# ak110/object_detector

Measured on AMD Instinct MI355X. Metric: images_per_sec, higher is better.
Workload: dtype f16

## Files before the change

object_detector_amd/csrc/conv_8ph_kernel.h:

```cpp
#pragma once
#include "conv_8ph_tile.h"
#include "conv_common.h"

namespace {

constexpr int E_ALO = 0, E_AHI = E_REGION, E_BLO = 2 * E_REGION, E_BHI = 3 * E_REGION;

struct TapWalk {
  int c0, tap, tapoff, dx;
  int sel_tap;
};

constexpr unsigned E_OOB = 0x80000000u;

template <int MT, int NF = 4, bool KEEP = false>
static __device__ __forceinline__ void e8_epilogue_rt(const ConvKP& p, f32x4 (&acc)[MT][NF], int m0w, int n0w, int l15,
                                                          int lq, f16x8 (*keep)[NF / 2] = nullptr, int mrows = MT * 16,
                                                          const float* pre_sc = nullptr, const float* pre_bi = nullptr) {
  unsigned pb[MT], ppix[MT];
#pragma unroll
  for (int i = 0; i < MT; ++i) {
    const int m = m0w + i * 16 + l15;
    pb[i] = (unsigned)m / (unsigned)p.HoWo;
    ppix[i] = (unsigned)m - pb[i] * (unsigned)p.HoWo;
  }
#pragma unroll
  for (int pr = 0; pr < NF / 2; ++pr) {
    const int n = n0w + (2 * pr + (lq & 1)) * 16 + (lq >> 1) * 8;
    const bool nok = n < p.Cout;
    float sc[8], bi[8];
    if (pre_sc) {
#pragma unroll
      for (int e = 0; e < 8; ++e) {
        sc[e] = pre_sc[e];
        bi[e] = pre_bi[e];
      }
    } else {
      const f32x4 s0 = *(const f32x4*)(p.scale + n), s1 = *(const f32x4*)(p.scale + n + 4);
      const f32x4 b0 = *(const f32x4*)(p.bias + n), b1 = *(const f32x4*)(p.bias + n + 4);
#pragma unroll
      for (int e = 0; e < 4; ++e) {
        sc[e] = s0[e];
        sc[4 + e] = s1[e];
        bi[e] = b0[e];
        bi[4 + e] = b1[e];
      }
    }
    f16x8 rv[MT];
#pragma unroll
    for (int i = 0; i < MT; ++i) {
      const int m = m0w + i * 16 + l15;
      f16x8 r = {0, 0, 0, 0, 0, 0, 0, 0};
      if (nok && m < p.M && p.res_mode != OD_RES_NONE) {
        long long roff;
        if (p.res_mode == OD_RES_SAME) {
          roff = (long long)m * p.Cout + n;
        } else {
          const unsigned ho = ppix[i] / (unsigned)p.Wo, wo = ppix[i] - ho * (unsigned)p.Wo;
          roff = ((long long)(pb[i] * (unsigned)(p.Ho >> 1) + (ho >> 1)) * (p.Wo >> 1) + (wo >> 1)) * p.Cout + n;
        }
        r = *(const f16x8*)(p.res + roff);
      }
      rv[i] = r;
    }
#pragma unroll
    for (int i = 0; i < MT; ++i) {
      const int m = m0w + i * 16 + l15;
      const bool ok = nok && m < p.M && i * 16 + l15 < mrows;
      float v[8];
#pragma unroll
      for (int e = 0; e < 4; ++e) {
        float a = acc[i][2 * pr][e], bq = acc[i][2 * pr + 1][e];
        od_permlane16_swap(a, bq);
        v[e] = a;
        v[4 + e] = bq;
      }
#pragma unroll
      for (int e = 0; e < 8; ++e) v[e] = v[e] * sc[e] + bi[e];
      if (p.act == OD_ACT_LEAKY) {
#pragma unroll
        for (int e = 0; e < 8; ++e) v[e] = od_leaky(v[e], p.alpha);
      } else if (p.act == OD_ACT_ELU) {
#pragma unroll
        for (int e = 0; e < 8; ++e) v[e] = v[e] > 0.f ? v[e] : p.alpha * od_expm1_fast(v[e]);
      }
      if (p.res_mode != OD_RES_NONE) {
#pragma unroll
        for (int e = 0; e < 8; ++e) v[e] += (float)rv[i][e];
      }
      if (ok) {
        const long long ooff = (long long)pb[i] * p.obs + (long long)ppix[i] * p.ops + n;
        if (p.out_f32) {
          float* o = (float*)p.out + ooff;
          *(f32x4*)o = f32x4{v[0], v[1], v[2], v[3]};
          *(f32x4*)(o + 4) = f32x4{v[4], v[5], v[6], v[7]};
        } else {
          f16x8 h;
#pragma unroll
          for (int e = 0; e < 8; ++e) h[e] = (f16)v[e];
          *(f16x8*)((f16*)p.out + ooff) = h;
        }
      }
      if (KEEP) {
        f16x8 h;
#pragma unroll
        for (int e = 0; e < 8; ++e) h[e] = (f16)v[e];
        keep[i][pr] = h;
      }
    }
  }
}

template <int EPI, int MT, int NF, bool KEEP>
static __device__ __forceinline__ void e8_epilogue_fixed(const ConvKP& p, f32x4 (&acc)[MT][NF], int m0w, int n0w, int l15, int lq,
                                                         f16x8 (*keep)[NF / 2], int mrows, const float* pre_sc,
                                                         const float* pre_bi) {
  constexpr int ACT = od_epi_act(EPI), RES = od_epi_res(EPI);
  constexpr bool F32 = od_epi_f32(EPI);
  unsigned orow[MT], rrow[RES != OD_RES_NONE ? MT : 1];
#pragma unroll
  for (int i = 0; i < MT; ++i) {
    const unsigned m = (unsigned)min(m0w + i * 16 + l15, p.M - 1);
    const unsigned b = m / (unsigned)p.HoWo, pix = m - b * (unsigned)p.HoWo;
    orow[i] = b * (unsigned)p.obs + pix * (unsigned)p.ops;
    if (RES == OD_RES_SAME) rrow[i] = m * (unsigned)p.Cout;
    if (RES == OD_RES_UP2) {
      const unsigned ho = pix / (unsigned)p.Wo, wo = pix - ho * (unsigned)p.Wo;
      rrow[i] = ((b * (unsigned)(p.Ho >> 1) + (ho >> 1)) * (unsigned)(p.Wo >> 1) + (wo >> 1)) * (unsigned)p.Cout;
    }
  }
#pragma unroll
  for (int pr = 0; pr < NF / 2; ++pr) {
    const int n = n0w + (2 * pr + (lq & 1)) * 16 + (lq >> 1) * 8;
    const bool nok = n < p.Cout;
    float sc[8], bi[8];
    if (pre_sc) {
#pragma unroll
      for (int e = 0; e < 8; ++e) {
        sc[e] = pre_sc[e];
        bi[e] = pre_bi[e];
      }
    } else {
      const f32x4 s0 = *(const f32x4*)(p.scale + n), s1 = *(const f32x4*)(p.scale + n + 4);
      const f32x4 b0 = *(const f32x4*)(p.bias + n), b1 = *(const f32x4*)(p.bias + n + 4);
#pragma unroll
      for (int e = 0; e < 4; ++e) {
        sc[e] = s0[e];
        sc[4 + e] = s1[e];
        bi[e] = b0[e];
        bi[4 + e] = b1[e];
      }
    }
    f16x8 rv[RES != OD_RES_NONE ? MT : 1];
    if (RES != OD_RES_NONE) {
      const unsigned nr = nok ? (unsigned)n : 0u;
#pragma unroll
      for (int i = 0; i < MT; ++i) rv[i] = *(const f16x8*)(p.res + (rrow[i] + nr));
    }
#pragma unroll
    for (int i = 0; i < MT; ++i) {
      f32x4 a = acc[i][2 * pr], bq = acc[i][2 * pr + 1];
      od_permlane16_swap4(a, bq);
      float v[8] = {a[0], a[1], a[2], a[3], bq[0], bq[1], bq[2], bq[3]};
#pragma unroll
      for (int e = 0; e < 8; ++e) v[e] = v[e] * sc[e] + bi[e];
      if (ACT == OD_ACT_LEAKY) {
#pragma unroll
        for (int e = 0; e < 8; ++e) v[e] = od_leaky(v[e], p.alpha);
      } else if (ACT == OD_ACT_ELU) {
#pragma unroll
        for (int e = 0; e < 8; ++e) v[e] = od_elu_select(v[e], p.alpha);
      }
      if (RES != OD_RES_NONE) {
#pragma unroll
        for (int e = 0; e < 8; ++e) v[e] += (float)rv[i][e];
      }
      f16x8 h;
      if (!F32 || KEEP) {
#pragma unroll
        for (int e = 0; e < 8; ++e) h[e] = (f16)v[e];
      }
      if (nok && m0w + i * 16 + l15 < p.M && i * 16 + l15 < mrows) {
        const unsigned ooff = orow[i] + (unsigned)n;
        if (F32) {
          float* o = (float*)p.out + ooff;
          *(f32x4*)o = f32x4{v[0], v[1], v[2], v[3]};
          *(f32x4*)(o + 4) = f32x4{v[4], v[5], v[6], v[7]};
        } else {
          *(f16x8*)((f16*)p.out + ooff) = h;
        }
      }
      if (KEEP) keep[i][pr] = h;
    }
  }
}

template <int MT, int NF = 4, bool KEEP = false, int EPI = OD_EPI_RT>
static __device__ __forceinline__ void e8_epilogue_direct(const ConvKP& p, f32x4 (&acc)[MT][NF], int m0w, int n0w, int l15,
                                                          int lq, f16x8 (*keep)[NF / 2] = nullptr, int mrows = MT * 16,
                                                          const float* pre_sc = nullptr, const float* pre_bi = nullptr) {
  if constexpr (EPI == OD_EPI_RT)
    e8_epilogue_rt<MT, NF, KEEP>(p, acc, m0w, n0w, l15, lq, keep, mrows, pre_sc, pre_bi);
  else
    e8_epilogue_fixed<EPI, MT, NF, KEEP>(p, acc, m0w, n0w, l15, lq, keep, mrows, pre_sc, pre_bi);
}

template <int KS, int MF1, int EPI, int EPI2, bool PW, bool SEG>
__global__ __launch_bounds__(512, 2) void od_conv_8ph(ConvKP p_in) {
  constexpr int MF0 = 4, MT = MF0 + MF1, WROWS = MT * 16, BM = 2 * WROWS;
  extern __shared__ __attribute__((aligned(16))) char smem[];
  const int tid = threadIdx.x;
  const int lane = tid & 63;
  const int wave = __builtin_amdgcn_readfirstlane(tid >> 6);
  const int wr = wave >> 2, wc = wave & 3;
  const int l15 = lane & 15, lq = lane >> 4;

  int logical;
  {
    const int nt = p_in.mtiles * p_in.ntiles;
    const int pid = p_in.splitk > 1 ? (int)blockIdx.x / p_in.splitk : (int)blockIdx.x;
    const int q = nt >> 3, r = nt & 7, xcd = pid & 7, loc = pid >> 3;
    logical = (xcd < r ? xcd * (q + 1) : r * (q + 1) + (xcd - r) * q) + loc;
  }
  int tm = logical / p_in.ntiles;
  const int tn = logical - tm * p_in.ntiles;
  ConvKP p_seg;
  if (SEG) p_seg = p_in;
  if (SEG && p_in.nseg > 1) {
    int sg = 0;
    if (tm >= p_in.seg_tile0[1]) sg = 1;
    if (p_in.nseg > 2 && tm >= p_in.seg_tile0[2]) sg = 2;
    tm -= p_in.seg_tile0[sg];
    p_seg.x = p_in.seg_x[sg];
    p_seg.out = p_in.seg_out[sg];
    p_seg.H = p_seg.Ho = p_in.seg_H[sg];
    p_seg.W = p_seg.Wo = p_in.seg_W[sg];
    p_seg.HoWo = p_seg.H * p_seg.W;
    p_seg.M = p_in.seg_M[sg];
    p_seg.x_bytes = (unsigned)p_seg.M * (unsigned)p_in.Cin * 2u;
    if (p_in.obs == 0) p_seg.obs = (long long)p_seg.HoWo * p_in.Cout;
  }
  const ConvKP& p = SEG ? p_seg : p_in;
  const int m0 = tm * BM, n0 = tn * E_BN;
  const int nk_all = p.Ktot / E_BK;
  const int ks0 = p.splitk > 1 ? ((int)blockIdx.x % p.splitk) * p.steps_per_split : 0;
  const int nk = p.splitk > 1 ? min(p.steps_per_split, nk_all - ks0) : nk_all;
  if (nk <= 0) return;

  const int rr = tid >> 3;
  const int lc = (tid & 7) ^ (rr & 7);
  int a_base[2][2];
  unsigned a_vmask[2][2];
  unsigned a_sel[2][2];
#pragma unroll
  for (int s = 0; s < 2; ++s)
#pragma unroll
    for (int j = 0; j < 2; ++j) {
      const int m = m0 + j * WROWS + s * 64 + rr;
      a_vmask[s][j] = 0u;
      a_base[s][j] = 0;
      if (m < p.M && (s == 0 || rr < MF1 * 16)) {
        const unsigned b = (unsigned)m / (unsigned)p.HoWo;
        const unsigned pix = (unsigned)m - b * (unsigned)p.HoWo;
        const unsigned ho = pix / (unsigned)p.Wo;
        const unsigned wo = pix - ho * (unsigned)p.Wo;
        const int hi0 = (int)ho * p.stride - p.pad, wi0 = (int)wo * p.stride - p.pad;
        a_base[s][j] = ((((int)b * p.H + hi0 + p.pad) * p.W + wi0 + p.pad) * p.Cin + lc * 8) * 2;
#pragma unroll
        for (int t = 0; t < KS * KS; ++t) {
          const int hi = hi0 + t / KS, wi = wi0 + t % KS;
          if ((unsigned)hi < (unsigned)p.H && (unsigned)wi < (unsigned)p.W) a_vmask[s][j] |= 1u << t;
        }
      }
    }
  int w_off[2][2];
#pragma unroll
  for (int s = 0; s < 2; ++s)
#pragma unroll
    for (int j = 0; j < 2; ++j) {
      const int n = n0 + (2 * j + (rr >> 5)) * 64 + s * 32 + (rr & 31);
      w_off[s][j] = (n * p.Kstride + lc * 8 + ks0 * E_BK) * 2;
    }
  const __amdgpu_buffer_rsrc_t rs_x = __builtin_amdgcn_make_buffer_rsrc(
      (void*)(p.x - (long long)p.pad * (p.W + 1) * p.Cin), 0, (int)(p.x_bytes + (unsigned)(p.pad * (p.W + 1) * p.Cin * 2)),
      0x00020000);
  const __amdgpu_buffer_rsrc_t rs_w = __builtin_amdgcn_make_buffer_rsrc((void*)p.w, 0, (int)p.w_bytes, 0x00020000);
  auto blds16 = [&](const __amdgpu_buffer_rsrc_t& rs, unsigned voff, int soff, char* lptr) {
    __builtin_amdgcn_raw_ptr_buffer_load_lds(rs, (__attribute__((address_space(3))) void*)lptr, 16, (int)voff, soff, 0, 0);
  };

  auto walk_init = [&](TapWalk& w, int kt) {
    const int k0 = kt * E_BK;
    if (KS == 3) {
      w.sel_tap = -1;
      w.tap = k0 / p.Cin;
      w.c0 = k0 - w.tap * p.Cin;
      const int dy = w.tap / 3;
      w.dx = w.tap - dy * 3;
      w.tapoff = (dy * p.W + w.dx) * p.Cin;
    } else {
      w.sel_tap = -1;
      w.tap = 0;
      w.c0 = k0;
      w.dx = 0;
      w.tapoff = 0;
    }
  };
  auto walk_next = [&](TapWalk& w) {
    w.c0 += E_BK;
    if (KS == 3 && w.c0 >= p.Cin) {
      w.c0 = 0;
      ++w.tap;
      if (++w.dx == 3) {
        w.dx = 0;
        w.tapoff += (p.W - 2) * p.Cin;
      } else {
        w.tapoff += p.Cin;
      }
    }
  };
  TapWalk walk_lo, walk_hi;
  walk_init(walk_lo, ks0);
  walk_init(walk_hi, ks0);

  char* const piece = smem + wave * 1024;
  auto stage_a = [&](int s, TapWalk& w, int buf) {
    const int koff = w.tapoff + w.c0;
    char* dst = piece + buf * E_BUF + (s ? E_AHI : E_ALO);
    if (w.sel_tap != w.tap) {
      w.sel_tap = w.tap;
#pragma unroll
      for (int j = 0; j < 2; ++j) a_sel[s][j] = ((a_vmask[s][j] >> w.tap) & 1u) ? (unsigned)a_base[s][j] : E_OOB;
    }
#pragma unroll
    for (int j = 0; j < 2; ++j) blds16(rs_x, a_sel[s][j], koff * 2, dst + j * 8192);
    walk_next(w);
  };
  auto stage_b = [&](int s, int t, int buf) {
    char* dst = piece + buf * E_BUF + (s ? E_BHI : E_BLO);
#pragma unroll
    for (int j = 0; j < 2; ++j) blds16(rs_w, (unsigned)w_off[s][j], t * (E_BK * 2), dst + j * 8192);
  };

  const int w2buf = ((nk - 1) & 1) ^ 1;
  const __amdgpu_buffer_rsrc_t rs_w2 =
      __builtin_amdgcn_make_buffer_rsrc((void*)(PW ? p.w2 : p.w), 0, (int)(PW ? p.w2_bytes : p.w_bytes), 0x00020000);
  auto stage_w2 = [&](int ks) {
#pragma unroll
    for (int h = 0; h < 2; ++h)
      blds16(rs_w2, (unsigned)(((h * 64 + rr) * p.K2stride + lc * 8) * 2), ks * (E_BK * 2),
             piece + w2buf * E_BUF + ks * E_REGION + h * 8192);
  };

  f32x4 acc[MT][4];
#pragma unroll
  for (int i = 0; i < MT; ++i)
#pragma unroll
    for (int j = 0; j < 4; ++j) acc[i][j] = f32x4{0.f, 0.f, 0.f, 0.f};

  stage_a(0, walk_lo, 0);
  stage_b(0, 0, 0);
  stage_b(1, 0, 0);
  stage_a(1, walk_hi, 0);
  if (nk > 1) {
    stage_a(0, walk_lo, 1);
    stage_b(0, 1, 1);
    wait_vmcnt<8>();
  } else {
    wait_vmcnt<0>();
  }
  __builtin_amdgcn_s_barrier();

  const int fa = (wr * 64 + l15) * 128 + ((lq ^ (l15 & 7)) * 16);
  const int fb = (wc * 32 + l15) * 128 + ((lq ^ (l15 & 7)) * 16);

  f16x8 xa[MF0][2], wlo[2][2], whi[2][2];
  auto ldf = [&](f16x8& dst, const char* src) { dst = *(const f16x8*)src; };
  auto mma = [&](f32x4& c, const f16x8& a, const f16x8& b) {
    c = __builtin_amdgcn_mfma_f32_16x16x32_f16(a, b, c, 0, 0, 0);
  };

  auto L0 = [&](int t) {
    const char* cur = smem + (t & 1) * E_BUF;
#pragma unroll
    for (int f = 0; f < 2; ++f)
#pragma unroll
      for (int kh = 0; kh < 2; ++kh) ldf(wlo[f][kh], cur + E_BLO + ((fb + f * 2048) ^ (kh * 64)));
#pragma unroll
    for (int f = 0; f < MF0; ++f)
#pragma unroll
      for (int kh = 0; kh < 2; ++kh) ldf(xa[f][kh], cur + E_ALO + ((fa + f * 2048) ^ (kh * 64)));
    if (t + 1 < nk) {
      stage_b(1, t + 1, (t & 1) ^ 1);
      wait_vmcnt<8>();
    } else if (PW) {
      stage_w2(0);
      wait_vmcnt<2>();
    } else {
      wait_vmcnt<0>();
    }
  };
  auto L1 = [&](int t) {
    const char* cur = smem + (t & 1) * E_BUF;
#pragma unroll
    for (int f = 0; f < 2; ++f)
#pragma unroll
      for (int kh = 0; kh < 2; ++kh) ldf(whi[f][kh], cur + E_BHI + ((fb + f * 2048) ^ (kh * 64)));
    if (t + 1 < nk) {
      stage_a(1, walk_hi, (t & 1) ^ 1);
      wait_vmcnt<8>();
    } else if (PW) {
      stage_w2(1);
    } else {
      wait_vmcnt<0>();
    }
  };
  auto L2 = [&](int t) {
    const char* cur = smem + (t & 1) * E_BUF;
#pragma unroll
    for (int f = 0; f < MF1; ++f)
#pragma unroll
      for (int kh = 0; kh < 2; ++kh) ldf(xa[f][kh], cur + E_AHI + ((fa + f * 2048) ^ (kh * 64)));
    if (t + 2 < nk) stage_a(0, walk_lo, t & 1);
    if (PW && t + 1 == nk) stage_w2(2);
  };
  auto L3 = [&](int t) {
    if (t + 2 < nk) {
      stage_b(0, t + 2, t & 1);
      wait_vmcnt<8>();
    } else if (PW && t + 1 == nk) {
      stage_w2(3);
    } else {
      wait_vmcnt<0>();
    }
  };
  auto M = [&](int ph) {
    __builtin_amdgcn_s_setprio(1);
#pragma unroll
    for (int kh = 0; kh < 2; ++kh)
#pragma unroll
      for (int i = 0; i < ((ph < 2) ? MF0 : MF1); ++i)
#pragma unroll
        for (int j = 0; j < 2; ++j) {
          if (ph == 0) mma(acc[i][j], wlo[j][kh], xa[i][kh]);
          if (ph == 1) mma(acc[i][2 + j], whi[j][kh], xa[i][kh]);
          if (ph == 2) mma(acc[MF0 + i][2 + j], whi[j][kh], xa[i][kh]);
          if (ph == 3) mma(acc[MF0 + i][j], wlo[j][kh], xa[i][kh]);
        }
    __builtin_amdgcn_s_setprio(0);
  };

  if (wr == 0) {
    for (int t = 0; t < nk; ++t) {
      L0(t);
      M(0);
      __builtin_amdgcn_s_barrier();
      L1(t);
      M(1);
      __builtin_amdgcn_s_barrier();
      L2(t);
      M(2);
      __builtin_amdgcn_s_barrier();
      L3(t);
      M(3);
      __builtin_amdgcn_s_barrier();
    }
  } else {
    L0(0);
    __builtin_amdgcn_s_barrier();
    for (int t = 0; t < nk; ++t) {
      M(0);
      L1(t);
      __builtin_amdgcn_s_barrier();
      M(1);
      L2(t);
      __builtin_amdgcn_s_barrier();
      M(2);
      L3(t);
      __builtin_amdgcn_s_barrier();
      M(3);
      if (t + 1 < nk) {
        L0(t + 1);
        __builtin_amdgcn_s_barrier();
      }
    }
  }
  __syncthreads();

  if constexpr (PW) {
    const int rg = wave >> 2, cg = wave & 3;
    float sc2[8], bi2[8];
    {
      const int n2 = cg * 32 + (lq & 1) * 16 + (lq >> 1) * 8;
      const f32x4 s0 = *(const f32x4*)(p.scale2 + n2), s1 = *(const f32x4*)(p.scale2 + n2 + 4);
      const f32x4 b0 = *(const f32x4*)(p.bias2 + n2), b1 = *(const f32x4*)(p.bias2 + n2 + 4);
#pragma unroll
      for (int e = 0; e < 4; ++e) {
        sc2[e] = s0[e];
        sc2[4 + e] = s1[e];
        bi2[e] = b0[e];
        bi2[4 + e] = b1[e];
      }
    }
    f16x8 ykeep[MT][2];
    od_mfma_results_ready();
    e8_epilogue_direct<MT, 4, true, EPI>(p, acc, m0 + wr * WROWS, n0 + wc * 64, l15, lq, ykeep);
    ConvKP p2 = p;
    p2.scale = p.scale2;
    p2.bias = p.bias2;
    p2.act = p.act2;
    p2.alpha = p.alpha2;
    p2.res_mode = OD_RES_NONE;
    p2.out = (void*)p.out2;
    p2.out_f32 = 0;
    p2.Cout = p.Cout2;
    p2.obs = (long long)p.HoWo * p.Cout2;
    p2.ops = p.Cout2;
    char* const ybuf = smem + (w2buf ^ 1) * E_BUF;
    const char* const wbuf = smem + w2buf * E_BUF;
    const int fy = (rg * 64 + l15) * 128 + ((lq ^ (l15 & 7)) * 16);
    const int fw = (cg * 32 + l15) * 128 + ((lq ^ (l15 & 7)) * 16);
#pragma unroll
    for (int half = 0; half < 2; ++half) {
      if (wr == half) {
#pragma unroll
        for (int i = 0; i < MT; ++i)
#pragma unroll
          for (int pr = 0; pr < 2; ++pr) {
            const int row = i * 16 + l15;
            const int chunk = (2 * pr + (lq & 1)) * 2 + (lq >> 1);
            *(f16x8*)(ybuf + wc * E_REGION + row * 128 + ((chunk ^ (row & 7)) * 16)) = ykeep[i][pr];
          }
      }
      asm volatile("s_waitcnt lgkmcnt(0)" ::: "memory");
      __builtin_amdgcn_s_barrier();
      f32x4 acc2[4][2];
#pragma unroll
      for (int i = 0; i < 4; ++i)
#pragma unroll
        for (int f = 0; f < 2; ++f) acc2[i][f] = f32x4{0.f, 0.f, 0.f, 0.f};
#pragma unroll
      for (int ks = 0; ks < 4; ++ks)
#pragma unroll
        for (int kh = 0; kh < 2; ++kh) {
          f16x8 wf[2], yf[4];
#pragma unroll
          for (int f = 0; f < 2; ++f) wf[f] = *(const f16x8*)(wbuf + ks * E_REGION + ((fw + f * 2048) ^ (kh * 64)));
#pragma unroll
          for (int i = 0; i < 4; ++i) yf[i] = *(const f16x8*)(ybuf + ks * E_REGION + ((fy + i * 2048) ^ (kh * 64)));
#pragma unroll
          for (int i = 0; i < 4; ++i)
#pragma unroll
            for (int f = 0; f < 2; ++f) acc2[i][f] = __builtin_amdgcn_mfma_f32_16x16x32_f16(wf[f], yf[i], acc2[i][f], 0, 0, 0);
        }
      od_mfma_results_ready();
      e8_epilogue_direct<4, 2, false, EPI2>(p2, acc2, m0 + half * WROWS + rg * 64, cg * 32, l15, lq, nullptr, WROWS - rg * 64, sc2, bi2);
      if (half == 0) {
        asm volatile("s_waitcnt lgkmcnt(0)" ::: "memory");
        __builtin_amdgcn_s_barrier();
      }
    }
  } else if (EPI == OD_EPI_RT && p.splitk > 1) {
    conv_epilogue<E_BN, 2, 4, MT, 4, 512>(p, smem, acc, m0, n0, tid, wr, wc, l15, lq);
  } else {
    od_mfma_results_ready();
    e8_epilogue_direct<MT, 4, false, EPI>(p, acc, m0 + wr * WROWS, n0 + wc * 64, l15, lq);
  }
}

}
```

Before: 22640.

## Interleave global-to-LDS staging into MFMA phases and overlap epilogue with last tile

Splits the buffer-to-LDS staging calls into per-piece issues and places them at fixed slots inside the MFMA loops, guarded by sched_barrier, so loads are spread between matrix instructions instead of issued in bursts. The main loop is specialised into steady, penultimate and last-iteration modes to remove runtime branches. For fixed non-upsample epilogues, scale, bias and residual loads and the output stores are issued per quarter during the final tile, overlapping epilogue work with the remaining MFMAs. The tap walk becomes branchless and the cached per-tap selector is dropped. This adds scheduling complexity and register pressure, and could hurt occupancy.

```diff
diff --git a/object_detector_amd/csrc/conv_8ph_kernel.h b/object_detector_amd/csrc/conv_8ph_kernel.h
--- a/object_detector_amd/csrc/conv_8ph_kernel.h
+++ b/object_detector_amd/csrc/conv_8ph_kernel.h
@@ -8,7 +8,6 @@
 
 struct TapWalk {
   int c0, tap, tapoff, dx;
-  int sel_tap;
 };
 
 constexpr unsigned E_OOB = 0x80000000u;
@@ -111,87 +110,117 @@
   }
 }
 
+template <int EPI, int N>
+struct E8RowOff {
+  unsigned orow[N], rrow[od_epi_res(EPI) != OD_RES_NONE ? N : 1];
+};
+template <int EPI, int N>
+struct E8PairIn {
+  float sc[8], bi[8];
+  f16x8 rv[od_epi_res(EPI) != OD_RES_NONE ? N : 1];
+};
+template <int EPI, int N, bool OUT = true>
+static __device__ __forceinline__ void e8_row_offsets(const ConvKP& p, int m0r, int l15, E8RowOff<EPI, N>& ro) {
+  constexpr int RES = od_epi_res(EPI);
+#pragma unroll
+  for (int i = 0; i < N; ++i) {
+    const unsigned m = (unsigned)min(m0r + i * 16 + l15, p.M - 1);
+    const unsigned b = m / (unsigned)p.HoWo, pix = m - b * (unsigned)p.HoWo;
+    if (OUT) ro.orow[i] = b * (unsigned)p.obs + pix * (unsigned)p.ops;
+    if (RES == OD_RES_SAME) ro.rrow[i] = m * (unsigned)p.Cout;
+    if (RES == OD_RES_UP2) {
+      const unsigned ho = pix / (unsigned)p.Wo, wo = pix - ho * (unsigned)p.Wo;
+      ro.rrow[i] = ((b * (unsigned)(p.Ho >> 1) + (ho >> 1)) * (unsigned)(p.Wo >> 1) + (wo >> 1)) * (unsigned)p.Cout;
+    }
+  }
+}
+template <int EPI, int N>
+static __device__ __forceinline__ void e8_pair_loads(const ConvKP& p, int n, const E8RowOff<EPI, N>& ro, const float* pre_sc,
+                                                     const float* pre_bi, E8PairIn<EPI, N>& in) {
+  constexpr int RES = od_epi_res(EPI);
+  if (pre_sc) {
+#pragma unroll
+    for (int e = 0; e < 8; ++e) {
+      in.sc[e] = pre_sc[e];
+      in.bi[e] = pre_bi[e];
+    }
+  } else {
+    const unsigned nb = (unsigned)n * 4u;
+    const f32x4 s0 = *(const f32x4*)((const char*)p.scale + nb), s1 = *(const f32x4*)((const char*)p.scale + (nb + 16u));
+    const f32x4 b0 = *(const f32x4*)((const char*)p.bias + nb), b1 = *(const f32x4*)((const char*)p.bias + (nb + 16u));
+#pragma unroll
+    for (int e = 0; e < 4; ++e) {
+      in.sc[e] = s0[e];
+      in.sc[4 + e] = s1[e];
+      in.bi[e] = b0[e];
+      in.bi[4 + e] = b1[e];
+    }
+  }
+  if (RES != OD_RES_NONE) {
+    const unsigned nr = n < p.Cout ? (unsigned)n : 0u;
+#pragma unroll
+    for (int i = 0; i < N; ++i) in.rv[i] = *(const f16x8*)((const char*)p.res + (ro.rrow[i] + nr) * 2u);
+  }
+}
+template <int EPI, int N, bool KEEP, int MT, int NF>
+static __device__ __forceinline__ void e8_pair_finish(const ConvKP& p, f32x4 (&acc)[MT][NF], int i0, int pr, int m0w, int n,
+                                                      int l15, f16x8 (*keep)[NF / 2], int mrows, const E8RowOff<EPI, N>& ro,
+                                                      const E8PairIn<EPI, N>& in) {
+  constexpr int ACT = od_epi_act(EPI), RES = od_epi_res(EPI);
+  constexpr bool F32 = od_epi_f32(EPI);
+  const bool nok = n < p.Cout;
+#pragma unroll
+  for (int i = 0; i < N; ++i) {
+    f32x4 a = acc[i0 + i][2 * pr], bq = acc[i0 + i][2 * pr + 1];
+    od_permlane16_swap4(a, bq);
+    float v[8] = {a[0], a[1], a[2], a[3], bq[0], bq[1], bq[2], bq[3]};
+#pragma unroll
+    for (int e = 0; e < 8; ++e) v[e] = v[e] * in.sc[e] + in.bi[e];
+    if (ACT == OD_ACT_LEAKY) {
+#pragma unroll
+      for (int e = 0; e < 8; ++e) v[e] = od_leaky(v[e], p.alpha);
+    } else if (ACT == OD_ACT_ELU) {
+#pragma unroll
+      for (int e = 0; e < 8; ++e) v[e] = od_elu_select(v[e], p.alpha);
+    }
+    if (RES != OD_RES_NONE) {
+#pragma unroll
+      for (int e = 0; e < 8; ++e) v[e] += (float)in.rv[i][e];
+    }
+    f16x8 h;
+    if (!F32 || KEEP) {
+#pragma unroll
+      for (int e = 0; e < 8; ++e) h[e] = (f16)v[e];
+    }
+    if (nok && m0w + (i0 + i) * 16 + l15 < p.M && (i0 + i) * 16 + l15 < mrows) {
+      const unsigned ooff = ro.orow[i] + (unsigned)n;
+      if (F32) {
+        float* o = (float*)p.out + ooff;
+        *(f32x4*)o = f32x4{v[0], v[1], v[2], v[3]};
+        *(f32x4*)(o + 4) = f32x4{v[4], v[5], v[6], v[7]};
+      } else {
+        *(f16x8*)((char*)p.out + ooff * 2u) = h;
+      }
+    }
+    if (KEEP) keep[i0 + i][pr] = h;
+  }
+}
+static __device__ __forceinline__ int e8_pair_channel(int n0w, int pr, int lq) {
+  return n0w + (2 * pr + (lq & 1)) * 16 + (lq >> 1) * 8;
+}
+
 template <int EPI, int MT, int NF, bool KEEP>
 static __device__ __forceinline__ void e8_epilogue_fixed(const ConvKP& p, f32x4 (&acc)[MT][NF], int m0w, int n0w, int l15, int lq,
                                                          f16x8 (*keep)[NF / 2], int mrows, const float* pre_sc,
                                                          const float* pre_bi) {
-  constexpr int ACT = od_epi_act(EPI), RES = od_epi_res(EPI);
-  constexpr bool F32 = od_epi_f32(EPI);
-  unsigned orow[MT], rrow[RES != OD_RES_NONE ? MT : 1];
-#pragma unroll
-  for (int i = 0; i < MT; ++i) {
-    const unsigned m = (unsigned)min(m0w + i * 16 + l15, p.M - 1);
-    const unsigned b = m / (unsigned)p.HoWo, pix = m - b * (unsigned)p.HoWo;
-    orow[i] = b * (unsigned)p.obs + pix * (unsigned)p.ops;
-    if (RES == OD_RES_SAME) rrow[i] = m * (unsigned)p.Cout;
-    if (RES == OD_RES_UP2) {
-      const unsigned ho = pix / (unsigned)p.Wo, wo = pix - ho * (unsigned)p.Wo;
-      rrow[i] = ((b * (unsigned)(p.Ho >> 1) + (ho >> 1)) * (unsigned)(p.Wo >> 1) + (wo >> 1)) * (unsigned)p.Cout;
-    }
-  }
+  E8RowOff<EPI, MT> ro;
+  e8_row_offsets<EPI, MT>(p, m0w, l15, ro);
 #pragma unroll
   for (int pr = 0; pr < NF / 2; ++pr) {
-    const int n = n0w + (2 * pr + (lq & 1)) * 16 + (lq >> 1) * 8;
-    const bool nok = n < p.Cout;
-    float sc[8], bi[8];
-    if (pre_sc) {
-#pragma unroll
-      for (int e = 0; e < 8; ++e) {
-        sc[e] = pre_sc[e];
-        bi[e] = pre_bi[e];
-      }
-    } else {
-      const f32x4 s0 = *(const f32x4*)(p.scale + n), s1 = *(const f32x4*)(p.scale + n + 4);
-      const f32x4 b0 = *(const f32x4*)(p.bias + n), b1 = *(const f32x4*)(p.bias + n + 4);
-#pragma unroll
-      for (int e = 0; e < 4; ++e) {
-        sc[e] = s0[e];
-        sc[4 + e] = s1[e];
-        bi[e] = b0[e];
-        bi[4 + e] = b1[e];
-      }
-    }
-    f16x8 rv[RES != OD_RES_NONE ? MT : 1];
-    if (RES != OD_RES_NONE) {
-      const unsigned nr = nok ? (unsigned)n : 0u;
-#pragma unroll
-      for (int i = 0; i < MT; ++i) rv[i] = *(const f16x8*)(p.res + (rrow[i] + nr));
-    }
-#pragma unroll
-    for (int i = 0; i < MT; ++i) {
-      f32x4 a = acc[i][2 * pr], bq = acc[i][2 * pr + 1];
-      od_permlane16_swap4(a, bq);
-      float v[8] = {a[0], a[1], a[2], a[3], bq[0], bq[1], bq[2], bq[3]};
-#pragma unroll
-      for (int e = 0; e < 8; ++e) v[e] = v[e] * sc[e] + bi[e];
-      if (ACT == OD_ACT_LEAKY) {
-#pragma unroll
-        for (int e = 0; e < 8; ++e) v[e] = od_leaky(v[e], p.alpha);
-      } else if (ACT == OD_ACT_ELU) {
-#pragma unroll
-        for (int e = 0; e < 8; ++e) v[e] = od_elu_select(v[e], p.alpha);
-      }
-      if (RES != OD_RES_NONE) {
-#pragma unroll
-        for (int e = 0; e < 8; ++e) v[e] += (float)rv[i][e];
-      }
-      f16x8 h;
-      if (!F32 || KEEP) {
-#pragma unroll
-        for (int e = 0; e < 8; ++e) h[e] = (f16)v[e];
-      }
-      if (nok && m0w + i * 16 + l15 < p.M && i * 16 + l15 < mrows) {
-        const unsigned ooff = orow[i] + (unsigned)n;
-        if (F32) {
-          float* o = (float*)p.out + ooff;
-          *(f32x4*)o = f32x4{v[0], v[1], v[2], v[3]};
-          *(f32x4*)(o + 4) = f32x4{v[4], v[5], v[6], v[7]};
-        } else {
-          *(f16x8*)((f16*)p.out + ooff) = h;
-        }
-      }
-      if (KEEP) keep[i][pr] = h;
-    }
+    const int n = e8_pair_channel(n0w, pr, lq);
+    E8PairIn<EPI, MT> in;
+    e8_pair_loads<EPI, MT>(p, n, ro, pre_sc, pre_bi, in);
+    e8_pair_finish<EPI, MT, KEEP>(p, acc, 0, pr, m0w, n, l15, keep, mrows, ro, in);
   }
 }
 
@@ -251,7 +280,6 @@
   const int lc = (tid & 7) ^ (rr & 7);
   int a_base[2][2];
   unsigned a_vmask[2][2];
-  unsigned a_sel[2][2];
 #pragma unroll
   for (int s = 0; s < 2; ++s)
 #pragma unroll
@@ -292,31 +320,28 @@
   auto walk_init = [&](TapWalk& w, int kt) {
     const int k0 = kt * E_BK;
     if (KS == 3) {
-      w.sel_tap = -1;
       w.tap = k0 / p.Cin;
       w.c0 = k0 - w.tap * p.Cin;
       const int dy = w.tap / 3;
       w.dx = w.tap - dy * 3;
       w.tapoff = (dy * p.W + w.dx) * p.Cin;
     } else {
-      w.sel_tap = -1;
       w.tap = 0;
       w.c0 = k0;
       w.dx = 0;
       w.tapoff = 0;
     }
   };
-  auto walk_next = [&](TapWalk& w) {
+  const int tap_row_step = (p.W - 2) * p.Cin;
+  auto walk_next = [&](TapWalk& w) __attribute__((always_inline)) {
     w.c0 += E_BK;
-    if (KS == 3 && w.c0 >= p.Cin) {
-      w.c0 = 0;
-      ++w.tap;
-      if (++w.dx == 3) {
-        w.dx = 0;
-        w.tapoff += (p.W - 2) * p.Cin;
-      } else {
-        w.tapoff += p.Cin;
-      }
+    if (KS == 3) {
+      const bool wrap = w.c0 >= p.Cin;
+      const bool row = wrap && w.dx == 2;
+      w.c0 = wrap ? 0 : w.c0;
+      w.tap += wrap ? 1 : 0;
+      w.tapoff += row ? tap_row_step : wrap ? p.Cin : 0;
+      w.dx = row ? 0 : w.dx + (wrap ? 1 : 0);
     }
   };
   TapWalk walk_lo, walk_hi;
@@ -324,32 +349,29 @@
   walk_init(walk_hi, ks0);
 
   char* const piece = smem + wave * 1024;
-  auto stage_a = [&](int s, TapWalk& w, int buf) {
-    const int koff = w.tapoff + w.c0;
-    char* dst = piece + buf * E_BUF + (s ? E_AHI : E_ALO);
-    if (w.sel_tap != w.tap) {
-      w.sel_tap = w.tap;
-#pragma unroll
-      for (int j = 0; j < 2; ++j) a_sel[s][j] = ((a_vmask[s][j] >> w.tap) & 1u) ? (unsigned)a_base[s][j] : E_OOB;
-    }
-#pragma unroll
-    for (int j = 0; j < 2; ++j) blds16(rs_x, a_sel[s][j], koff * 2, dst + j * 8192);
+  auto stage_a_piece = [&](int s, const TapWalk& w, int buf, int j) __attribute__((always_inline)) {
+    const unsigned sel = ((a_vmask[s][j] >> w.tap) & 1u) ? (unsigned)a_base[s][j] : E_OOB;
+    blds16(rs_x, sel, (w.tapoff + w.c0) * 2, piece + buf * E_BUF + (s ? E_AHI : E_ALO) + j * 8192);
+  };
+  auto stage_b_piece = [&](int s, int t, int buf, int j) __attribute__((always_inline)) {
+    blds16(rs_w, (unsigned)w_off[s][j], t * (E_BK * 2), piece + buf * E_BUF + (s ? E_BHI : E_BLO) + j * 8192);
+  };
+  auto stage_a = [&](int s, TapWalk& w, int buf) __attribute__((always_inline)) {
+    stage_a_piece(s, w, buf, 0);
+    stage_a_piece(s, w, buf, 1);
     walk_next(w);
   };
-  auto stage_b = [&](int s, int t, int buf) {
-    char* dst = piece + buf * E_BUF + (s ? E_BHI : E_BLO);
-#pragma unroll
-    for (int j = 0; j < 2; ++j) blds16(rs_w, (unsigned)w_off[s][j], t * (E_BK * 2), dst + j * 8192);
+  auto stage_b = [&](int s, int t, int buf) __attribute__((always_inline)) {
+    stage_b_piece(s, t, buf, 0);
+    stage_b_piece(s, t, buf, 1);
   };
 
   const int w2buf = ((nk - 1) & 1) ^ 1;
   const __amdgpu_buffer_rsrc_t rs_w2 =
       __builtin_amdgcn_make_buffer_rsrc((void*)(PW ? p.w2 : p.w), 0, (int)(PW ? p.w2_bytes : p.w_bytes), 0x00020000);
-  auto stage_w2 = [&](int ks) {
-#pragma unroll
-    for (int h = 0; h < 2; ++h)
-      blds16(rs_w2, (unsigned)(((h * 64 + rr) * p.K2stride + lc * 8) * 2), ks * (E_BK * 2),
-             piece + w2buf * E_BUF + ks * E_REGION + h * 8192);
+  auto stage_w2_piece = [&](int ks, int h) __attribute__((always_inline)) {
+    blds16(rs_w2, (unsigned)(((h * 64 + rr) * p.K2stride + lc * 8) * 2), ks * (E_BK * 2),
+           piece + w2buf * E_BUF + ks * E_REGION + h * 8192);
   };
 
   f32x4 acc[MT][4];
@@ -375,117 +397,189 @@
   const int fb = (wc * 32 + l15) * 128 + ((lq ^ (l15 & 7)) * 16);
 
   f16x8 xa[MF0][2], wlo[2][2], whi[2][2];
-  auto ldf = [&](f16x8& dst, const char* src) { dst = *(const f16x8*)src; };
-  auto mma = [&](f32x4& c, const f16x8& a, const f16x8& b) {
+  auto ldf = [&](f16x8& dst, const char* src) __attribute__((always_inline)) { dst = *(const f16x8*)src; };
+  auto mma = [&](f32x4& c, const f16x8& a, const f16x8& b) __attribute__((always_inline)) {
     c = __builtin_amdgcn_mfma_f32_16x16x32_f16(a, b, c, 0, 0, 0);
   };
 
-  auto L0 = [&](int t) {
+  constexpr int T_STEADY = 0;
+  constexpr int T_PENULT = 1;
+  constexpr int T_LAST = 2;
+  auto R = [&](int ph, int t) __attribute__((always_inline)) {
     const char* cur = smem + (t & 1) * E_BUF;
-#pragma unroll
-    for (int f = 0; f < 2; ++f)
-#pragma unroll
-      for (int kh = 0; kh < 2; ++kh) ldf(wlo[f][kh], cur + E_BLO + ((fb + f * 2048) ^ (kh * 64)));
-#pragma unroll
-    for (int f = 0; f < MF0; ++f)
-#pragma unroll
-      for (int kh = 0; kh < 2; ++kh) ldf(xa[f][kh], cur + E_ALO + ((fa + f * 2048) ^ (kh * 64)));
-    if (t + 1 < nk) {
-      stage_b(1, t + 1, (t & 1) ^ 1);
+    if (ph == 0) {
+#pragma unroll
+      for (int f = 0; f < 2; ++f)
+#pragma unroll
+        for (int kh = 0; kh < 2; ++kh) ldf(wlo[f][kh], cur + E_BLO + ((fb + f * 2048) ^ (kh * 64)));
+#pragma unroll
+      for (int f = 0; f < MF0; ++f)
+#pragma unroll
+        for (int kh = 0; kh < 2; ++kh) ldf(xa[f][kh], cur + E_ALO + ((fa + f * 2048) ^ (kh * 64)));
+    }
+    if (ph == 1) {
+#pragma unroll
+      for (int f = 0; f < 2; ++f)
+#pragma unroll
+        for (int kh = 0; kh < 2; ++kh) ldf(whi[f][kh], cur + E_BHI + ((fb + f * 2048) ^ (kh * 64)));
+    }
+    if (ph == 2) {
+#pragma unroll
+      for (int f = 0; f < MF1; ++f)
+#pragma unroll
+        for (int kh = 0; kh < 2; ++kh) ldf(xa[f][kh], cur + E_AHI + ((fa + f * 2048) ^ (kh * 64)));
+    }
+  };
+  auto D = [&](int ph, int mode, int t, int j) __attribute__((always_inline)) {
+    if (mode == T_LAST) {
+      if (PW) stage_w2_piece(ph, j);
+      return;
+    }
+    if (ph == 0) stage_b_piece(1, t + 1, (t & 1) ^ 1, j);
+    if (ph == 1) {
+      stage_a_piece(1, walk_hi, (t & 1) ^ 1, j);
+      if (j == 1) walk_next(walk_hi);
+    }
+    if (mode == T_STEADY && ph == 2) {
+      stage_a_piece(0, walk_lo, t & 1, j);
+      if (j == 1) walk_next(walk_lo);
+    }
+    if (mode == T_STEADY && ph == 3) stage_b_piece(0, t + 2, t & 1, j);
+  };
+  auto W = [&](int ph, int mode) __attribute__((always_inline)) {
+    if (mode == T_LAST) {
+      if (ph == 0) {
+        if (PW)
+          wait_vmcnt<2>();
+        else
+          wait_vmcnt<0>();
+      }
+    } else if (ph == 0 || ph == 1 || (ph == 3 && mode == T_STEADY)) {
       wait_vmcnt<8>();
-    } else if (PW) {
-      stage_w2(0);
-      wait_vmcnt<2>();
-    } else {
+    } else if (ph == 3) {
       wait_vmcnt<0>();
     }
   };
-  auto L1 = [&](int t) {
-    const char* cur = smem + (t & 1) * E_BUF;
-#pragma unroll
-    for (int f = 0; f < 2; ++f)
-#pragma unroll
-      for (int kh = 0; kh < 2; ++kh) ldf(whi[f][kh], cur + E_BHI + ((fb + f * 2048) ^ (kh * 64)));
-    if (t + 1 < nk) {
-      stage_a(1, walk_hi, (t & 1) ^ 1);
-      wait_vmcnt<8>();
-    } else if (PW) {
-      stage_w2(1);
-    } else {
-      wait_vmcnt<0>();
-    }
-  };
-  auto L2 = [&](int t) {
-    const char* cur = smem + (t & 1) * E_BUF;
-#pragma unroll
-    for (int f = 0; f < MF1; ++f)
-#pragma unroll
-      for (int kh = 0; kh < 2; ++kh) ldf(xa[f][kh], cur + E_AHI + ((fa + f * 2048) ^ (kh * 64)));
-    if (t + 2 < nk) stage_a(0, walk_lo, t & 1);
-    if (PW && t + 1 == nk) stage_w2(2);
-  };
-  auto L3 = [&](int t) {
-    if (t + 2 < nk) {
-      stage_b(0, t + 2, t & 1);
-      wait_vmcnt<8>();
-    } else if (PW && t + 1 == nk) {
-      stage_w2(3);
-    } else {
-      wait_vmcnt<0>();
-    }
-  };
-  auto M = [&](int ph) {
+  auto M = [&](int ph, int dph, int dmode, int dt) __attribute__((always_inline)) {
+    const int rows = (ph < 2) ? MF0 : MF1;
+    const int slot0 = rows, slot1 = (5 * rows) / 2;
+    int n = 0;
     __builtin_amdgcn_s_setprio(1);
 #pragma unroll
     for (int kh = 0; kh < 2; ++kh)
 #pragma unroll
-      for (int i = 0; i < ((ph < 2) ? MF0 : MF1); ++i)
+      for (int i = 0; i < rows; ++i)
 #pragma unroll
         for (int j = 0; j < 2; ++j) {
+          if (dph >= 0 && (n == slot0 || n == slot1)) {
+            __builtin_amdgcn_sched_barrier(0);
+            D(dph, dmode, dt, n == slot0 ? 0 : 1);
+            __builtin_amdgcn_sched_barrier(0);
+          }
           if (ph == 0) mma(acc[i][j], wlo[j][kh], xa[i][kh]);
           if (ph == 1) mma(acc[i][2 + j], whi[j][kh], xa[i][kh]);
           if (ph == 2) mma(acc[MF0 + i][2 + j], whi[j][kh], xa[i][kh]);
           if (ph == 3) mma(acc[MF0 + i][j], wlo[j][kh], xa[i][kh]);
+          ++n;
         }
     __builtin_amdgcn_s_setprio(0);
   };
 
-  if (wr == 0) {
-    for (int t = 0; t < nk; ++t) {
-      L0(t);
-      M(0);
+  constexpr bool EARLY = !PW && EPI != OD_EPI_RT && od_epi_res(EPI) != OD_RES_UP2;
+  constexpr int EPIQ = EARLY ? EPI : OD_EPI_LINEAR_NONE_F32;
+  E8RowOff<EPIQ, MF0> q_lo;
+  E8RowOff<EPIQ, MF1> q_hi;
+  E8PairIn<EPIQ, MF0> q_in_lo;
+  E8PairIn<EPIQ, MF1> q_in_hi;
+  const int m0w = m0 + wr * WROWS, n0w = n0 + wc * 64;
+  auto Q_loads = [&](int q) __attribute__((always_inline)) {
+    if constexpr (EARLY) {
+      if (q == 0) e8_row_offsets<EPIQ, MF0, false>(p, m0w, l15, q_lo);
+      if (q == 2) e8_row_offsets<EPIQ, MF1, false>(p, m0w + MF0 * 16, l15, q_hi);
+      const int n = e8_pair_channel(n0w, (q == 1 || q == 2) ? 1 : 0, lq);
+      if (q < 2)
+        e8_pair_loads<EPIQ, MF0>(p, n, q_lo, nullptr, nullptr, q_in_lo);
+      else
+        e8_pair_loads<EPIQ, MF1>(p, n, q_hi, nullptr, nullptr, q_in_hi);
+    }
+  };
+  auto Q_store = [&](int q) __attribute__((always_inline)) {
+    if constexpr (EARLY) {
+      const int pr = (q == 1 || q == 2) ? 1 : 0;
+      const int n = e8_pair_channel(n0w, pr, lq);
+      if (q == 0) e8_row_offsets<EPIQ, MF0>(p, m0w, l15, q_lo);
+      if (q == 2) e8_row_offsets<EPIQ, MF1>(p, m0w + MF0 * 16, l15, q_hi);
+      od_mfma_results_ready();
+      if (q < 2)
+        e8_pair_finish<EPIQ, MF0, false>(p, acc, 0, pr, m0w, n, l15, nullptr, MT * 16, q_lo, q_in_lo);
+      else
+        e8_pair_finish<EPIQ, MF1, false>(p, acc, MF0, pr, m0w, n, l15, nullptr, MT * 16, q_hi, q_in_hi);
+    }
+  };
+
+  auto tile_row0 = [&](int t, int mode) __attribute__((always_inline)) {
+#pragma unroll
+    for (int ph = 0; ph < 4; ++ph) {
+      R(ph, t);
+      M(ph, ph, mode, t);
+      if (mode == T_LAST && ph > 0) Q_store(ph - 1);
+      W(ph, mode);
+      if (mode == T_LAST) Q_loads(ph);
       __builtin_amdgcn_s_barrier();
-      L1(t);
-      M(1);
+    }
+  };
+  auto tile_row1 = [&](int t, int mode) __attribute__((always_inline)) {
+#pragma unroll
+    for (int ph = 0; ph < 3; ++ph) {
+      M(ph, ph + 1, mode, t);
+      if (mode == T_LAST && ph > 0) Q_store(ph - 1);
+      if (mode == T_LAST) Q_loads(ph);
+      R(ph + 1, t);
+      W(ph + 1, mode);
       __builtin_amdgcn_s_barrier();
-      L2(t);
-      M(2);
+    }
+    if (mode != T_LAST) {
+      const int next = mode == T_STEADY ? T_PENULT : T_LAST;
+      M(3, 0, next, t + 1);
+      R(0, t + 1);
+      W(0, next);
       __builtin_amdgcn_s_barrier();
-      L3(t);
-      M(3);
+    } else {
+      M(3, -1, mode, t);
+      Q_store(2);
+      Q_loads(3);
+    }
+  };
+  {
+    int t = 0;
+    if (wr == 0) {
+      for (; t + 2 < nk; ++t) tile_row0(t, T_STEADY);
+      if (t + 1 < nk) tile_row0(t++, T_PENULT);
+      tile_row0(t, T_LAST);
+    } else {
+      if (nk > 1) {
+        D(0, T_PENULT, 0, 0);
+        D(0, T_PENULT, 0, 1);
+        R(0, 0);
+        W(0, T_PENULT);
+      } else {
+        D(0, T_LAST, 0, 0);
+        D(0, T_LAST, 0, 1);
+        R(0, 0);
+        W(0, T_LAST);
+      }
       __builtin_amdgcn_s_barrier();
-    }
+      for (; t + 2 < nk; ++t) tile_row1(t, T_STEADY);
+      if (t + 1 < nk) tile_row1(t++, T_PENULT);
+      tile_row1(t, T_LAST);
+    }
+  }
+  if constexpr (EARLY) {
+    Q_store(3);
+    return;
   } else {
-    L0(0);
-    __builtin_amdgcn_s_barrier();
-    for (int t = 0; t < nk; ++t) {
-      M(0);
-      L1(t);
-      __builtin_amdgcn_s_barrier();
-      M(1);
-      L2(t);
-      __builtin_amdgcn_s_barrier();
-      M(2);
-      L3(t);
-      __builtin_amdgcn_s_barrier();
-      M(3);
-      if (t + 1 < nk) {
-        L0(t + 1);
-        __builtin_amdgcn_s_barrier();
-      }
-    }
-  }
-  __syncthreads();
+    __syncthreads();
+  }
 
   if constexpr (PW) {
     const int rg = wave >> 2, cg = wave & 3;
```

Result: no change. 22870, median of 6 (+1.0%).
